# FYTalon/pienerf

Hardware: AMD Instinct MI355X
Metric: sim+render steps/s @800x800 chair (higher is better)
Workload: dtype f32 render / f64 sim

## Files before the change

### include/pienerf_hip.h

```cpp
#ifndef PIENERF_HIP_H
#define PIENERF_HIP_H
#include <stdint.h>
#ifdef __cplusplus
extern "C" {
#endif

#define PN_OK 0
#define PN_ERR_ARG 1
#define PN_ERR_HIP 2
#define PN_ERR_CAPACITY 3

const char* pn_version(void);

int pn_stream_create_cu_mask(uint32_t total_cu, uint32_t first_cu, uint32_t n_cu, int invert, void** stream_out);
int pn_stream_destroy(void* stream);
int pn_march_set_tail_rounds(int rounds);
int pn_march_set_skip_dda(int on);
int pn_device_cu_count(void);
const char* pn_last_error(void);


int pn_sph_from_ray(const float* rays_o, const float* rays_d, float radius, uint32_t N, float* coords, void* stream);
int pn_near_far_from_aabb(const float* rays_o, const float* rays_d, const float* aabb, uint32_t N, float min_near, float* nears, float* fars,
                          void* stream);
// ... 106 lines not shown
    float IP_dx;
    int cut;
    float cut_bounds[6];
    float bound;
    float min_near;
    float dt_gamma;
    uint32_t max_steps;
    float T_thresh;
    uint32_t cascade;
    uint32_t grid_size;
    float density_scale;
    float bg_color;
    int fp16;
    int reuse_tables;
    int ray_batch;
    int throughput;
    int throughput_trips;
    int ray_tile_w;
    int fused_from;
    int fused_whole;
    int fused_fold;
    int fused_grid;
    int fused_order;
} pn_render_opts;
int pn_frame_create(pn_frame** out, uint32_t max_rays, uint32_t max_vtx, uint32_t max_grid_cells);
void pn_frame_destroy(pn_frame* f);
int pn_render_deformed(pn_frame* f, const pn_net* net, const pn_render_opts* opts, const float* rays_o, const float* rays_d, uint32_t N,
                       const float* p_def, const float* p_ori, const float* F_IP, const float* dF_IP, int n_vtx, const uint8_t* bitfield,
                       float* image, float* depth, float* depth_0, float* weights_sum, int64_t* stats_host, void* stream);

int pn_render_deformed_async(pn_frame* f, const pn_net* net, const pn_render_opts* opts, const float* rays_o, const float* rays_d, uint32_t N,
                             const float* p_def, const float* p_ori, const float* F_IP, const float* dF_IP, int n_vtx, const uint8_t* bitfield,
                             float* image, float* depth, float* depth_0, float* weights_sum, int n_trips, void* stream);
int pn_render_status(pn_frame* f, int64_t* stats_host, int synchronize, void* stream);
int pn_frame_reset_unfinished(pn_frame* f, void* stream);

int pn_render_continue(pn_frame* f, const pn_net* net, const pn_render_opts* opts, const float* rays_o, const float* rays_d, uint32_t N,
                       const uint8_t* bitfield, float* image, float* depth, float* depth_0, float* weights_sum, int64_t* stats_host, int n_trips,
                       int is_static, void* stream);

int pn_render_static(pn_frame* f, const pn_net* net, const pn_render_opts* opts, const float* rays_o, const float* rays_d, uint32_t N,
                     const float* aabb_host, const uint8_t* bitfield, float* image, float* depth, float* depth_0, float* weights_sum,
                     int64_t* stats_host, int n_trips, void* stream);


typedef struct pn_copier pn_copier;
int pn_copier_create(pn_copier** out);
void pn_copier_destroy(pn_copier* c);
int pn_copier_submit(pn_copier* c, void* dst_host, const void* src_dev, uint64_t bytes, void* after_event, uint64_t* ticket);
int pn_copier_wait(pn_copier* c, uint64_t ticket);


int pn_mark_untrained_grid(const float* poses, uint32_t B, float fx, float fy, float cx, float cy, uint32_t cascade, uint32_t H, float bound,
                           float* density_grid, int* n_unseen, void* stream);
int pn_density_cells_full(uint32_t cascade, uint32_t H, float bound, const float* noise, float* xyzs, void* stream);
int pn_density_cells_partial(uint32_t cas, uint32_t H, float bound, uint32_t N, const int* rand_coords, const float* rand_pick, const float* noise,
                             const float* density_grid_cas, float* tmp_grid_cas, int* scratch, int* indices, float* xyzs, void* stream);
uint64_t pn_density_partial_scratch_ints(uint32_t H);
int pn_density_scatter(uint32_t n, const int* indices, const float* sigmas, float* tmp_grid_cas, void* stream);
int pn_density_grid_update(uint32_t n, float* density_grid, const float* tmp_grid, float decay, float density_thresh, uint8_t* bitfield,
                           double* partial, float* mean_thresh, void* stream);

int pn_frame_march_counters(pn_frame* f, int enable, uint64_t* counters_host, void* stream);
int pn_frame_fused_clocks(pn_frame* f, uint64_t* clocks_host, int* first_trip_out, int reset, void* stream);
int pn_fused_order_host(const float* rays_t, const float* fars, int n_rays, int* perm_out);
int pn_frame_trip_records(pn_frame* f, int* records_host, int* tail_counts_host, int max_trips, void* stream);
int pn_frame_trip_times(pn_frame* f, float* march_ms_host, float* network_ms_host, int max_trips, int* n_trips_out, void* stream);


int pn_sim_update_F(int n_IP, const int* topo, const double* dof, const double* Nx, const double* dNx, const double* ddNx, float* pos, float* F,
                    float* dF, void* stream);

int pn_sim_calc_elastic(int n_IP, const int* topo, const double* dNx, const double* dof, double* RF, double* VF, double* FF, int mcadams_sweeps,
                        void* stream);

int pn_sim_collect_rhs(int n_k, double dx, const int* csr_bg, const int* csr_cnt, const int* csr_buf, const double* mu, const double* lam,
                       const double* dNx, const double* RF, const double* VF, double* rhs, void* stream);

int pn_sim_matvec3(int n, const double* A, const double* X, double* Y, void* stream);

int pn_sim_stepforward(int n_k, int n_IP, int iters, double dt, double dx, const int* topo, const int* csr_bg, const int* csr_cnt,
                       const int* csr_buf, const double* mu, const double* lam, const double* dNx, const double* dNx_csr, const int* csr_pos,
                       const double* Ainv,
                       const double* Mmat, const double* dof_rest, const double* rhs_rest, const double* rhs_gravity, const double* dof_f,
                       double* dof, double* dof_vel, double* work, int prepared, int mcadams_sweeps, void* stream);
uint64_t pn_sim_work_doubles(int n_k, int n_IP);
int pn_sim_cells_chunk_ips(void);
// ... 248 lines not shown
```

### pienerf_amd/_lib.py

```python
import ctypes as C
import os

_HERE = os.path.dirname(os.path.abspath(__file__))
LIB_PATH = os.environ.get("PN_LIB_PATH") or os.path.join(_HERE, "lib", "libpienerf_hip.so")

P = C.c_void_p
u32, i32, f32, f64, u64 = C.c_uint32, C.c_int, C.c_float, C.c_double, C.c_uint64


class RenderOpts(C.Structure):
    _fields_ = [("max_iter_num", i32), ("hash_grid_size", f32), ("num_seek_IP", i32), ("IP_dx", f32), ("cut", i32), ("cut_bounds", f32 * 6),
                ("bound", f32), ("min_near", f32), ("dt_gamma", f32), ("max_steps", u32), ("T_thresh", f32), ("cascade", u32), ("grid_size", u32),
                ("density_scale", f32), ("bg_color", f32), ("fp16", i32), ("reuse_tables", i32), ("ray_batch", i32), ("throughput", i32), ("throughput_trips", i32), ("ray_tile_w", i32),
                ("fused_from", i32), ("fused_whole", i32), ("fused_fold", i32), ("fused_grid", i32), ("fused_order", i32)]


class ColliderStyle(C.Structure):
    _fields_ = [("rgb", (f32 * 3) * 8), ("checker", f32), ("checker_dim", f32), ("ambient", f32)]


class ShadowLight(C.Structure):
    _fields_ = [("c", f32 * 3), ("L", f32 * 3), ("U", f32 * 3), ("V", f32 * 3), ("half", f32), ("D", f32), ("S", i32), ("strength", f32), ("bias", f32),
                ("spheres", i32)]


class PointStyle(C.Structure):
    _fields_ = [("radius", i32), ("mode", i32), ("xray", i32), ("rgb", f32 * 3), ("ramp", (f32 * 3) * 3), ("lo", f32), ("hi", f32), ("alpha", f32),
                ("hidden_alpha", f32), ("bias", f32), ("marker_radius", f32), ("marker_thickness", f32)]


SIGNATURES = {
    "pn_version": (C.c_char_p, []),
    "pn_last_error": (C.c_char_p, []),
    "pn_stream_create_cu_mask": (i32, [u32, u32, u32, i32, C.POINTER(C.c_void_p)]),
    "pn_stream_destroy": (i32, [P]),
    "pn_device_cu_count": (i32, []),
    "pn_march_set_tail_rounds": (i32, [i32]),
# ... 43 lines not shown
    "pn_background_coords": (i32, [P, P, P, u32, P, i32, P]),
    "pn_nerf_color": (i32, [P, P, P, P, u32, P, P]),
    "pn_nerf_color_half": (i32, [P, P, P, P, u32, P, P]),
    "pn_render_hier": (i32, [P, P, P, u32, C.POINTER(f32), f32, i32, i32, f32, f32, P, P, P, P, i32, P]),
    "pn_hier_max_samples": (i32, []),
    "pn_frame_create": (i32, [C.POINTER(P), u32, u32, u32]),
    "pn_frame_destroy": (None, [P]),
    "pn_render_deformed": (i32, [P, P, C.POINTER(RenderOpts), P, P, u32, P, P, P, P, i32, P, P, P, P, P, P, P]),
    "pn_render_deformed_async": (i32, [P, P, C.POINTER(RenderOpts), P, P, u32, P, P, P, P, i32, P, P, P, P, P, i32, P]),
    "pn_render_status": (i32, [P, P, i32, P]),
    "pn_frame_reset_unfinished": (i32, [P, P]),
    "pn_render_continue": (i32, [P, P, C.POINTER(RenderOpts), P, P, u32, P, P, P, P, P, P, i32, i32, P]),
    "pn_render_static": (i32, [P, P, C.POINTER(RenderOpts), P, P, u32, P, P, P, P, P, P, P, i32, P]),
    "pn_mark_untrained_grid": (i32, [P, u32, f32, f32, f32, f32, u32, u32, f32, P, P, P]),
    "pn_density_cells_full": (i32, [u32, u32, f32, P, P, P]),
    "pn_density_cells_partial": (i32, [u32, u32, f32, u32, P, P, P, P, P, P, P, P, P]),
    "pn_density_partial_scratch_ints": (u64, [u32]),
    "pn_density_scatter": (i32, [u32, P, P, P, P]),
    "pn_density_grid_update": (i32, [u32, P, P, f32, f32, P, P, P, P]),
    "pn_frame_march_counters": (i32, [P, i32, P, P]),
    "pn_frame_trip_times": (i32, [P, P, P, i32, P, P]),
    "pn_frame_fused_clocks": (i32, [P, P, P, i32, P]),
    "pn_fused_order_host": (i32, [P, P, i32, P]),
    "pn_net_form": (i32, [P]),
    "pn_net_form_epoch": (i32, [P]),
    "pn_frame_trip_records": (i32, [P, P, P, i32, P]),
    "pn_sim_update_F": (i32, [i32, P, P, P, P, P, P, P, P, P]),
    "pn_sim_calc_elastic": (i32, [i32, P, P, P, P, P, P, i32, P]),
    "pn_sim_collect_rhs": (i32, [i32, f64, P, P, P, P, P, P, P, P, P, P]),
    "pn_sim_matvec3": (i32, [i32, P, P, P, P]),
    "pn_sim_stepforward": (i32, [i32, i32, i32, f64, f64, P, P, P, P, P, P, P, P, P, P, P, P, P, P, P, P, P, P, i32, i32, P]),
    "pn_sim_prepare": (i32, [i32, i32, P, P, P, P]),
    "pn_sim_cells_chunk_ips": (i32, []),
    "pn_sim_cells_work_doubles": (u64, [i32, i32]),
    "pn_sim_cells_prepare": (i32, [i32, i32, P, P]),
    "pn_sim_stepforward_cells": (i32, [i32, i32, i32, f64, f64, P, P, P, P, P, P, P, P, P, P, P, P, P, P, P, i32, P]),
    "pn_sim_bsr_matvec3": (i32, [i32, P, P, P, P, P, P]),
    "pn_sim_pcg_work_doubles": (u64, [i32]),
    "pn_sim_pcg_solve": (i32, [i32, P, P, P, P, P, P, P, f64, i32, P, P, P]),
    "pn_sim_stepforward_cells_pcg": (i32, [i32, i32, i32, f64, f64, P, P, P, P, P, P, P, P, P, P, P, P, f64, i32, P, P, P, P, P, P, P, P, P, i32, P]),
    "pn_sim_work_doubles": (u64, [i32, i32]),
    "pn_sim_coop_bytes": (u64, [i32, i32, i32]),
    "pn_sim_coop_prepare": (i32, [i32, i32, i32, P, P, P, C.POINTER(i32), P]),
    "pn_sim_coop_status": (i32, [P, C.POINTER(i32)]),
    "pn_sim_stepforward_coop": (i32, [i32, i32, i32, f64, f64, P, P, P, P, P, P, P, P, P, P, P, P, P, P, P, P, i32, C.POINTER(i32), P]),
    "pn_sim_update_force": (i32, [i32, i32, P, f64, P, P, P, P, P]),
# ... 98 lines not shown
```

### pienerf_amd/csrc/pn_render_ops.hip

```cpp
#include <float.h>

#include <vector>

#include "pn_render_records.h"
#include "pn_cell_hash.h"
#include "pn_side_tables.h"
#include "pn_march_kernels.h"
#include "pn_composite.h"
#include "pn_compact.h"
#include "pn_frame_kernels.h"

thread_local char pn_err_buf[512] = {0};

extern "C" int pn_device_cu_count(void) {
    int dev = 0, n = 0;
    if (hipGetDevice(&dev) != hipSuccess) return -1;
    if (hipDeviceGetAttribute(&n, hipDeviceAttributeMultiprocessorCount, dev) != hipSuccess) return -1;
    return n;
}

extern "C" int pn_stream_create_cu_mask(uint32_t total_cu, uint32_t first_cu, uint32_t n_cu, int invert, void** stream_out) {
    PN_REQUIRE(stream_out && total_cu > 0 && total_cu <= 1024 && n_cu > 0 && first_cu + n_cu <= total_cu);
    uint32_t mask[32];
    const uint32_t words = (total_cu + 31) / 32;
// ... 433 lines not shown
    pn_frame* f = c.f;
    const pn_net* net = c.net;
    const pn_render_opts* o = c.o;
    const bool whole = form == 1, fold = form == 2;
    int rc;
    if (fold) {
        if ((rc = time_mark(f, c.st, 0, 0, true))) return rc;
        enqueue_march(c, pl, 0, false);
        f->head_marched = 1;
        if ((rc = time_mark(f, c.st, 0, 1, true)) || (rc = time_mark(f, c.st, 0, 2, true))) return rc;
    }
    FusedArgs fa;
    memset(&fa, 0, sizeof(fa));
    fa.lv = (const PnFusedLevel*)(o->fp16 ? net->fused_levels : net->byte_levels); fa.emb = net->embeddings; fa.emb_h = (const uint32_t*)net->emb_half; fa.emb_bytes = net->n_entries * 4u;
    fa.wimg_g = (const uint4*)(o->fp16 ? net->whalf : (net->x_ok ? net->wx : net->wsplit)); fa.net_bound = net->bound; fa.net_inv2b = 1.0f / (2 * net->bound); fa.density_scale = o->density_scale;
    fa.x_scales = net->x_scales;
    fa.trips = f->trips + t; fa.N_rays = c.N; fa.max_steps = o->max_steps; fa.T_thresh = o->T_thresh;
    fa.alive = alive_list(f, t);
    fa.rays_t = f->rays_t; fa.weights_sum = c.weights_sum; fa.depth = c.depth_0; fa.image = f->acc_image;
    fa.xyzs = f->xyzs; fa.dirs = f->dirs; fa.deltas = f->deltas; fa.sigmas = f->sigmas; fa.rgbs = f->rgbs;
    fa.ctl = f->fused_ctl; fa.dev = f->dev; fa.tail_diag = f->tail_counts + t;
    fa.clocks = (f->march_counters_on & 4) ? f->fused_clocks : nullptr;
    fa.order = o->fused_order >= 0 ? 1 : 0;
    if (whole) {
        fa.active = f->active_seg; fa.active_counts = seg_counter(f, SEG_ACTIVE); fa.active_seg_cap = (int)f->seg_cap; fa.t_resume = f->t_resume;
        fa.blist = f->blist; fa.strag = f->strag; fa.blist_cap = f->blist_cap;
        fa.a_rounds = 24;
    }
    if (fold) {
        fa.list_seg = f->list_seg; fa.samp_counts = seg_counter(f, SEG_SAMP); fa.list_seg_cap = (int)f->seg_cap;
        fa.seg_tail = seg_counter(f, SEG_TAIL); fa.seg_back = seg_counter(f, SEG_BACK);
        fa.blist = f->blist; fa.strag = f->strag; fa.blist_cap = f->blist_cap;
    }
    if (finalize) {
        fa.finalize = 1; fa.bg = o->bg_color; fa.nears = f->nears; fa.fars_full = f->fars; fa.image_out = c.image; fa.depth_out = c.depth;
    }
    const int tb_idx = fold ? 1 : t;
    if ((rc = time_mark(f, c.st, tb_idx, 0, true))) return rc;
    if (whole) enqueue_skip(c, pl, make_march_io(c, pl, 0));
    const uint32_t blocks = o->fused_grid > 0 ? std::min((uint32_t)o->fused_grid, f->fused_blocks) : f->fused_blocks;
    rc = launch_trips_fused(o->num_seek_IP, o->max_iter_num > 1, o->fp16 ? 1 : (net->x_ok ? 2 : 0), form, blocks, c.st, c.mq, c.tb, fa);
    if (rc) return rc;
    if ((rc = time_mark(f, c.st, tb_idx, 1, true)) || (rc = time_mark(f, c.st, tb_idx, 2, true))) return rc;
    f->fused_first = tb_idx;
    f->fused_mode = form;
    return PN_OK;
// ... 161 lines not shown
            fprintf(stderr, "\n");
        }
#endif
        PN_HIP_CHECK(hipStreamSynchronize(st));
    }
    if ((enable & 1) && !(f->march_counters_on & 1)) PN_HIP_CHECK(hipMemsetAsync(f->march_counters, 0, 16 * sizeof(unsigned long long), st));
    f->march_counters_on = enable & 7;
    return PN_OK;
}

extern "C" int pn_frame_fused_clocks(pn_frame* f, uint64_t* clocks_host, int* first_trip_out, int reset, void* stream) {
    PN_REQUIRE(f);
    hipStream_t st = (hipStream_t)stream;
    if (clocks_host) {
        PN_HIP_CHECK(hipMemcpyAsync(clocks_host, f->fused_clocks, 16 * sizeof(unsigned long long), hipMemcpyDeviceToHost, st));
        PN_HIP_CHECK(hipStreamSynchronize(st));
        clocks_host[15] = f->fused_first >= 0 ? (uint64_t)f->fused_mode : 0u;
    }
    if (first_trip_out) *first_trip_out = f->fused_first;
    if (reset) PN_HIP_CHECK(hipMemsetAsync(f->fused_clocks, 0, 16 * sizeof(unsigned long long), st));
    return PN_OK;
}

extern "C" int pn_fused_order_host(const float* rays_t, const float* fars, int n_rays, int* perm_out) {
    PN_REQUIRE(n_rays >= 0 && (n_rays == 0 || (rays_t && fars && perm_out)));
    const int n_packets = (n_rays + PN_ORDER_PACKET - 1) / PN_ORDER_PACKET;
    const int n_ord = std::min(n_packets, PN_ORDER_CAP);
    std::vector<float> keys((size_t)n_ord, 0.0f);
    for (int k = 0; k < n_ord; k++)
        for (int s = 0; s < PN_ORDER_PACKET && k * PN_ORDER_PACKET + s < n_rays; s++)
            keys[k] = fmaxf(keys[k], pn_order_key(rays_t[k * PN_ORDER_PACKET + s], fars[k * PN_ORDER_PACKET + s]));
    for (int k = 0; k < n_ord; k++) perm_out[pn_order_rank(keys.data(), n_ord, k)] = k;
    for (int k = n_ord; k < n_packets; k++) perm_out[k] = k;
    return PN_OK;
}

extern "C" int pn_frame_trip_times(pn_frame* f, float* march_ms_host, float* network_ms_host, int max_trips, int* n_trips_out, void* stream) {
    PN_REQUIRE(f && march_ms_host && network_ms_host && n_trips_out && max_trips >= 0);
    PN_HIP_CHECK(hipStreamSynchronize((hipStream_t)stream));
    const int n = f->timed_trips < max_trips ? f->timed_trips : max_trips;
    if (f->stamped) {
        static unsigned long long host[PN_TIMED_TRIPS * 3];
        PN_HIP_CHECK(hipMemcpy(host, f->stamps, sizeof(unsigned long long) * (size_t)n * 3, hipMemcpyDeviceToHost));
        for (int t = 0; t < n; t++) {
            march_ms_host[t] = (float)((double)(host[t * 3 + 1] - host[t * 3]) * 1e-5);
            network_ms_host[t] = (float)((double)(host[t * 3 + 2] - host[t * 3 + 1]) * 1e-5);
// ... 40 lines not shown
```

### pienerf_amd/csrc/pn_trips_fused.h

```cpp
#pragma once
#define PN_TU_FP_CONTRACT_OFF 1
#include <cstddef>

#include "pn_net_tile.h"
#include "pn_fused_order.h"

#define PN_FUSED_MAX_TRIPS 128
#if PN_DBG_PHASES
#define PN_FUSED_PK , pk_dummy_
#else
#define PN_FUSED_PK
#endif
#ifndef PN_FUSED_WROUNDS
#define PN_FUSED_WROUNDS 1
#endif
#ifndef PN_FUSED_WAVES
#define PN_FUSED_WAVES 12
#endif
#ifndef PN_FUSED_LDS_OUT
#define PN_FUSED_LDS_OUT 1
#endif
#ifndef PN_FUSED_LDS_XYZ
#define PN_FUSED_LDS_XYZ 1
#endif
#define PN_FUSED_STAGE 512
#define PN_FUSED_CTL_HIST 0
#define PN_FUSED_CTL_DONE (PN_FUSED_CTL_HIST + 3 * PN_FUSED_MAX_TRIPS)
#define PN_FUSED_CTL_INTS (PN_FUSED_CTL_DONE + 32)
// ... 7 lines not shown
    float net_bound, net_inv2b, density_scale;
    const float* x_scales;
    PnTrip* trips;
    uint32_t N_rays, max_steps;
    float T_thresh;
    const int* alive;
    float *rays_t, *weights_sum, *depth, *image;
    float *xyzs, *dirs, *deltas, *sigmas, *rgbs;
    int* ctl;
    PnFrameDev* dev;
    int* tail_diag;
    unsigned long long* clocks;
    const int* active;
    const int* active_counts;
    int active_seg_cap;
    const float* t_resume;
    int* blist;
    int4* strag;
    uint32_t blist_cap;
    int a_rounds;
    int finalize; float bg; const float* nears; const float* fars_full; float* image_out; float* depth_out;
    const int* list_seg; const int* samp_counts; int list_seg_cap; const int* seg_tail; const int* seg_back;
    int order;
};

#ifndef PN_FUSED_FRESH_ARGS
#define PN_FUSED_FRESH_ARGS 1
#endif
__device__ __forceinline__ constexpr size_t pn_align_up(size_t v, size_t a) { return (v + a - 1) / a * a; }
template <typename T, int WHICH>
__device__ __forceinline__ const T& fused_karg_fresh(const T& by_value) {
#if PN_FUSED_FRESH_ARGS
    struct Layout { pnm::MarchParams a; pnm2::March2Tables tb; FusedArgs fa; };
    constexpr size_t off_tb = pn_align_up(sizeof(pnm::MarchParams), alignof(pnm2::March2Tables));
    constexpr size_t off_fa = pn_align_up(off_tb + sizeof(pnm2::March2Tables), alignof(FusedArgs));
    static_assert(off_tb == offsetof(Layout, tb) && off_fa == offsetof(Layout, fa), "kernarg placement of (MarchParams, March2Tables, FusedArgs)");
    constexpr size_t off = WHICH == 0 ? 0 : (WHICH == 1 ? off_tb : off_fa);
    uint32_t z;
    asm volatile("s_mov_b32 %0, 0" : "=s"(z));
    const char __attribute__((address_space(4)))* kp = (const char __attribute__((address_space(4)))*)__builtin_amdgcn_kernarg_segment_ptr();
    return *reinterpret_cast<const T*>((const char*)kp + off + z);
#else
    return by_value;
#endif
}
__device__ __forceinline__ const FusedArgs& fused_args_fresh(const FusedArgs& by_value) { return fused_karg_fresh<FusedArgs, 2>(by_value); }
// ... 66 lines not shown
#define PN_FUSED_ACHUNK 64
#endif

template <int K, bool MULTI, int NF, int MODE>
__global__ void __launch_bounds__(PN_FUSED_WAVES * 64, (PN_FUSED_WAVES + 3) / 4) k_trips_fused(pnm::MarchParams a, pnm2::March2Tables tb, FusedArgs fa) {
    extern __shared__ __attribute__((aligned(16))) uint4 fused_lds[];
    constexpr bool HALF = NF == 1, XF = NF == 2;
    constexpr int IMG16 = (HALF ? PN_NET_HALF_BYTES : (XF ? PN_NET_X_BYTES : PN_NET_SPLIT_BYTES)) / 16;
    constexpr int MAXT = PN_FUSED_MAX_TRIPS;
    constexpr int AC = PN_FUSED_ACHUNK;
    static_assert(AC == 64 || AC == 32, "rays per first-trip chunk");
    constexpr bool WHOLE = MODE == 1;
    constexpr bool FOLD = MODE == 2;
    constexpr bool QUEUED = MODE != 0;
    uint4* wimg = fused_lds;
    float4* stage_all = reinterpret_cast<float4*>(fused_lds + IMG16 + 32);
    int* hist = reinterpret_cast<int*>(stage_all + PN_FUSED_WAVES * PN_FUSED_STAGE);
    constexpr bool LXYZ = PN_FUSED_LDS_XYZ != 0 && PN_FUSED_LDS_OUT != 0 && NF != 0;
    float* xyz_all = reinterpret_cast<float*>(hist + 3 * MAXT);
    __shared__ int s_last, s_cursor;
    __shared__ int s_bres, s_bready, s_bhead, s_sres, s_sready, s_shead, s_pending, s_a1done;
    __shared__ int s_pend[PN_FUSED_MAXCHUNKS];
    __shared__ int s_pref[PN_SEGS + 1];
    __shared__ unsigned short s_perm[PN_ORDER_CAP];

#if PN_DBG_PHASES
    pnm3::PhaseClock pk_dummy_;
#endif
    const PnTrip* tr = fa.trips;
    const int lane = threadIdx.x & 63, wv = threadIdx.x >> 6;
    if (PN_FUSED_FRESH_ARGS && blockIdx.x == 0 && threadIdx.x == 0) {
        const FusedArgs& fk = fused_args_fresh(fa);
        const pnm::MarchParams& ak = fused_karg_fresh<pnm::MarchParams, 0>(a);
        const pnm2::March2Tables& tk = fused_karg_fresh<pnm2::March2Tables, 1>(tb);
        if (fk.trips != fa.trips || fk.rays_t != fa.rays_t || fk.N_rays != fa.N_rays || fk.image_out != fa.image_out || fk.seg_back != fa.seg_back || ak.rays_o != a.rays_o ||
            ak.grid != a.grid || ak.hgs != a.hgs || tk.nb != tb.nb || tk.rec != tb.rec) atomicOr(&fa.dev->err, 32);
    }
    const float x_scale = XF ? fa.x_scales[0] : 1.0f, x_rscale = XF ? fa.x_scales[1] : 1.0f;
    int A = 0, sb0 = 0, n_active = 0;
    if (QUEUED) {
        if (threadIdx.x < 64) {
            const int cnt = seg_count(WHOLE ? fa.active_counts : fa.samp_counts, lane);
            int inc = cnt;
#pragma unroll
            for (int o = 1; o < 64; o <<= 1) {
                const int u = __shfl_up(inc, o);
                if (lane >= o) inc += u;
            }
            s_pref[lane + 1] = inc;
            if (lane == 0) s_pref[0] = 0;
        }
        __syncthreads();
        n_active = s_pref[PN_SEGS];
        const long long chunks = ((long long)n_active + AC - 1) / AC;
        const bool ok = tr->n_alive == (int)fa.N_rays && tr->n_step == 1 && tr->step_base == 0 && (long long)n_active * 8 <= (long long)fa.N_rays &&
                        (chunks + (long long)gridDim.x) * AC <= (long long)fa.blist_cap &&
                        (WHOLE ? (chunks + (long long)gridDim.x - 1) / (long long)gridDim.x <= PN_FUSED_MAXCHUNKS : true);
        if (!ok) return;
        sb0 = 1;
    } else {
        A = tr->n_alive; sb0 = tr->step_base;
        if (!(A > 0 && tr->n_step == 8 && tr->dense != 0)) return;
    }

    for (int i = threadIdx.x; i < IMG16; i += PN_FUSED_WAVES * 64) wimg[i] = fa.wimg_g[i];
    if (threadIdx.x < 16 * sizeof(PnFusedLevel) / 16) wimg[IMG16 + threadIdx.x] = reinterpret_cast<const uint4*>(fa.lv)[threadIdx.x];
    for (int i = threadIdx.x; i < 3 * MAXT; i += PN_FUSED_WAVES * 64) hist[i] = 0;
    if (threadIdx.x == 0) { s_cursor = 0; s_bres = s_bready = s_bhead = s_sres = s_sready = s_shead = s_a1done = 0; }
    if (QUEUED) {
        const int n_items0 = WHOLE ? (n_active + AC - 1) / AC : (n_active + 31) / 32;
        const int mine0 = (int)blockIdx.x < n_items0 ? (n_items0 - (int)blockIdx.x + (int)gridDim.x - 1) / (int)gridDim.x : 0;
        if (threadIdx.x == 0) s_pending = mine0;
        if (WHOLE)
            for (int i = threadIdx.x; i < PN_FUSED_MAXCHUNKS; i += PN_FUSED_WAVES * 64) s_pend[i] = 64;
    }
    __syncthreads();

    const int sub = lane & 7, gbase = lane & ~7, grp = lane >> 3;
    const uint32_t wave_g = blockIdx.x * PN_FUSED_WAVES + wv;
    const uint32_t slotw = (FOLD ? fa.N_rays : 0u) + wave_g * 64u, slot0 = slotw + (uint32_t)grp * 8u;
    float4* stage = stage_all + wv * PN_FUSED_STAGE;
    const uint4* __restrict__ wl = wimg + lane;
    const int half = lane >> 5, s32 = lane & 31;
    const PnFusedLevel* lds_lv = reinterpret_cast<const PnFusedLevel*>(wimg + IMG16) + 8 * half;
    __amdgpu_buffer_rsrc_t emb_rsrc = __builtin_amdgcn_make_buffer_rsrc(const_cast<uint32_t*>(fa.emb_h), 0, (int)fa.emb_bytes, 0x00020000);
    float* const X = LXYZ ? xyz_all + wv * 192 + grp * 24 : fa.xyzs + (size_t)slot0 * 3;
    float* const Dd = LXYZ ? nullptr : fa.dirs + (size_t)slot0 * 3;
    float* const dl = fa.deltas + (size_t)slot0 * 2;

    const bool clk = fa.clocks != nullptr;
    unsigned long long c_acc[10] = {0, 0, 0, 0, 0, 0, 0, 0, 0, 0}, c_t = 0, rounds = 0;
    auto tick = [&](int k) __attribute__((always_inline)) {
        if (clk) {
            asm volatile("s_waitcnt vmcnt(0) lgkmcnt(0)" ::: "memory");
            const unsigned long long n = __builtin_readcyclecounter();
            c_acc[k] += n - c_t;
            c_t = n;
        }
    };
    unsigned long long rt0 = 0;
    if (clk) { c_t = __builtin_readcyclecounter(); rt0 = __builtin_amdgcn_s_memrealtime(); }

    float r_ox = 0.f, r_oy = 0.f, r_oz = 0.f, r_dx = 1.f, r_dy = 1.f, r_dz = 1.f, r_rdx = 1.f, r_rdy = 1.f, r_rdz = 1.f, r_far = 0.f, r_t = 0.f;
    auto network_tile = [&](uint32_t slot, float4* lds_out = nullptr, const float* lds_xyz = nullptr, int dir_lane = 0) __attribute__((always_inline)) {
        pnm3::Float3 p, d;
        if (LXYZ && lds_xyz) {
            p = *reinterpret_cast<const pnm3::Float3*>(lds_xyz);
            d.x = __shfl(r_dx, dir_lane); d.y = __shfl(r_dy, dir_lane); d.z = __shfl(r_dz, dir_lane);
        } else {
            p = *reinterpret_cast<const pnm3::Float3*>(fa.xyzs + (size_t)slot * 3);
            d = *reinterpret_cast<const pnm3::Float3*>(fa.dirs + (size_t)slot * 3);
        }
        float sigma_logit, e[3];
        if (HALF) {
            float g2[8];
            tile_sigma_net_h<4>(fa.lv, wimg, emb_rsrc, wl, half, fa.net_bound, p.x, p.y, p.z, g2);
            sigma_logit = g2[0];
            __builtin_amdgcn_sched_barrier(0);
            tile_color_net_h(wl, wimg, half, g2, d.x, d.y, d.z, e);
        } else if (XF) {
            const f32x16 h2 = tile_sigma_net_x<PN_BF_LU>(reinterpret_cast<const PnByteLevel*>(lds_lv), fa.emb, wl, half, fa.net_bound, fa.net_inv2b, p.x, p.y, p.z, x_scale);
            sigma_logit = h2[0] * x_rscale;
            __builtin_amdgcn_sched_barrier(0);
            tile_color_net_x(wl, wimg, half, h2, d.x, d.y, d.z, e);
        } else {
            const f32x16 h2 = tile_sigma_net<PN_BF_LU>(reinterpret_cast<const PnByteLevel*>(lds_lv), fa.emb, wl, half, fa.net_bound, fa.net_inv2b, p.x, p.y, p.z);
            sigma_logit = h2[0];
            __builtin_amdgcn_sched_barrier(0);
            tile_color_net(wl, wimg, half, h2, d.x, d.y, d.z, e);
        }
        if (half == 0) {
            const float sg_ = tile_sigma_out(fa.density_scale, sigma_logit);
            const float c0_ = HALF ? tile_rgb_out_h(e[0]) : tile_rgb_out(e[0]), c1_ = HALF ? tile_rgb_out_h(e[1]) : tile_rgb_out(e[1]),
                        c2_ = HALF ? tile_rgb_out_h(e[2]) : tile_rgb_out(e[2]);
            if (lds_out) {
                *lds_out = make_float4(sg_, c0_, c1_, c2_);
            } else {
                fa.sigmas[slot] = sg_;
                fa.rgbs[(size_t)slot * 3] = c0_; fa.rgbs[(size_t)slot * 3 + 1] = c1_; fa.rgbs[(size_t)slot * 3 + 2] = c2_;
            }
        }
    };
    auto network64 = [&](unsigned long long rm, bool own = true, uint32_t lane_slot = 0u) __attribute__((always_inline)) {
#pragma unroll 1
        for (int tile = 0; tile < 2; tile++) {
            if (!((rm >> (32 * tile)) & 0xFFFFFFFFull)) continue;
            network_tile(own ? slotw + 32u * (uint32_t)tile + (uint32_t)s32 : lane_slot, (PN_FUSED_LDS_OUT && own) ? stage + 32 * tile + s32 : nullptr,
                         (LXYZ && own) ? xyz_all + wv * 192 + (32 * tile + s32) * 3 : nullptr, (4 * tile + (s32 >> 3)) * 8);
        }
    };
    auto wave_sync_mem = [&]() __attribute__((always_inline)) {
        __builtin_amdgcn_fence(__ATOMIC_RELEASE, "workgroup");
        asm volatile("s_waitcnt vmcnt(0)" ::: "memory");
        __builtin_amdgcn_fence(__ATOMIC_ACQUIRE, "workgroup");
    };

    int share = 0;
    const int* my_list = nullptr;
    int my_chunks = 0;
    int *a_index = nullptr, *blist = nullptr;
    int4* strag = nullptr;
    uint32_t a_base = 0;
    bool go_on = true;
    auto lds_ld = [](int* p_) __attribute__((always_inline)) { return __hip_atomic_load(p_, __ATOMIC_RELAXED, __HIP_MEMORY_SCOPE_WORKGROUP); };
    auto lds_st = [](int* p_, int v) __attribute__((always_inline)) { __hip_atomic_store(p_, v, __ATOMIC_RELAXED, __HIP_MEMORY_SCOPE_WORKGROUP); };
    auto q_claim = [&](int* head, int* ready, int want, int& take) __attribute__((always_inline)) {
        int base = 0;
        take = 0;
        for (;;) {
            const int h = lds_ld(head), r = lds_ld(ready);
            const int t_ = min(want, r - h);
            if (t_ <= 0) break;
            if (atomicCAS(head, h, h + t_) == h) { base = h; take = t_; break; }
        }
        return base;
    };
    auto q_publish = [&](int* ready, int base, int n) __attribute__((always_inline)) {
        while (lds_ld(ready) != base) __builtin_amdgcn_s_sleep(1);
        lds_st(ready, base + n);
    };
    auto chunk_finish = [&](int ci) __attribute__((always_inline)) {
#pragma unroll 1
        for (int tile = 0; tile < AC / 32; tile++) {
            const int pos = ci * AC + tile * 32 + s32;
            const uint32_t slot = a_base + (uint32_t)pos;
            const bool has = fa.deltas[(size_t)slot * 2] != 0.0f;
            const unsigned long long em = __ballot(has && half == 0);
            if (!em) continue;
            if (lane == 0) {
                atomicAdd(&hist[MAXT], (int)__popcll(em));
                if (a.stats) atomicAdd(a.stats + 3, (unsigned long long)__popcll(em));
            }
            network_tile(slot);
            wave_sync_mem();
            tick(7);
            bool on = false;
            int idx = -1;
            if (has && half == 0) {
                idx = a_index[pos];
                on = composite_one(idx, slot, 1u, fa.T_thresh, fa.rays_t, fa.sigmas, fa.rgbs, fa.deltas, fa.weights_sum, fa.depth, fa.image) && go_on;
                if (!on && fa.finalize) finalize_ray(fa, idx);
            }
            const unsigned long long om = __ballot(on);
            wave_sync_mem();
            if (om) {
                int base = 0;
                if (lane == 0) base = atomicAdd(&s_bres, (int)__popcll(om));
                base = __builtin_amdgcn_readfirstlane(base);
                if (on) blist[base + (int)__popcll(om & ((1ull << lane) - 1ull))] = idx;
                wave_sync_mem();
                if (lane == 0) q_publish(&s_bready, base, (int)__popcll(om));
            }
            tick(8);
        }
        if (lane == 0) atomicSub(&s_pending, 1);
// ... 174 lines not shown
                    f_has = e < n_active;
                    if (f_has) {
                        int lo = 0, hi = PN_SEGS;
                        while (hi - lo > 1) {
                            const int mid = (lo + hi) >> 1;
                            if (s_pref[mid] <= e) lo = mid; else hi = mid;
                        }
                        f_slot = (uint32_t)fa.list_seg[(size_t)lo * fa.list_seg_cap + (e - s_pref[lo])];
                    }
                    f_slot = f_has ? f_slot : (uint32_t)__builtin_amdgcn_readlane((int)f_slot, (int)__builtin_ctzll(__ballot(f_has)));
                }
            }
            if (!fold_round) {
                int fin = 0;
                if (lane == 0) fin = (lds_ld(&s_pending) == 0 && lds_ld(&s_bhead) >= lds_ld(&s_bready)) ? 1 : 0;
                if (__builtin_amdgcn_readfirstlane(fin)) break;
                __builtin_amdgcn_s_sleep(32);
                tick(9);
                continue;
            }
        }
        unsigned long long net_mask = 0ull;
        bool have_ray = false;
        if (fold_round) {
            net_mask = __ballot(f_has && half == 0);
            if (lane == 0) atomicAdd(&hist[MAXT], (int)__popcll(net_mask));
            tick(0);
        } else {
        rounds++;
        tick(0);
        have_ray = index >= 0;
        if (have_ray && sub == 0) atomicAdd(&hist[j], 1);
        const pnm::MarchParams& am = fused_karg_fresh<pnm::MarchParams, 0>(a);
        const pnm2::March2Tables& tbm = fused_karg_fresh<pnm2::March2Tables, 1>(tb);
        pnm3::RayConsts c;
        pnm3::frame_consts(am, c);
        c.ox = r_ox; c.oy = r_oy; c.oz = r_oz; c.dx = r_dx; c.dy = r_dy; c.dz = r_dz; c.rdx = r_rdx; c.rdy = r_rdy; c.rdz = r_rdz; c.far = r_far;
        pnm3::RayState st{0.f, 0.f, 0u};
        bool have = false;
        if (have_ray) {
            float t = r_t;
            t += pnm::clampf(t * am.dt_gamma, c.dt_min, c.dt_max) * 0.0f;
            st.last_t = t;
            st.t = t;
            have = t < c.far;
        }
        const bool done = pnm3::march_window<K, MULTI, 8, PN_FUSED_STAGE, 1>(am, tbm, c, 8u, sub, gbase, lane, stage, X, Dd, dl, st, PN_FUSED_WROUNDS, have PN_FUSED_PK);
        const bool deferred = have && !done;
// ... 7 lines not shown
            pnm3::frame_consts(am, c2);
            c2.ox = readlane_f(c.ox, L); c2.oy = readlane_f(c.oy, L); c2.oz = readlane_f(c.oz, L);
            c2.dx = readlane_f(c.dx, L); c2.dy = readlane_f(c.dy, L); c2.dz = readlane_f(c.dz, L);
            c2.rdx = readlane_f(c.rdx, L); c2.rdy = readlane_f(c.rdy, L); c2.rdz = readlane_f(c.rdz, L);
            c2.far = readlane_f(c.far, L);
            pnm3::RayState s2{readlane_f(st.t, L), readlane_f(st.last_t, L), (uint32_t)__builtin_amdgcn_readlane((int)st.step, L)};
            const size_t sl = (size_t)slotw + (size_t)(L >> 3) * 8;
            pnm3::march_window<K, MULTI, 64, PN_FUSED_STAGE, 1>(am, tbm, c2, 8u, lane, 0, lane, stage, LXYZ ? xyz_all + wv * 192 + (L >> 3) * 24 : fa.xyzs + sl * 3,
                                                                LXYZ ? nullptr : fa.dirs + sl * 3, fa.deltas + sl * 2, s2, 0x7fffffff, true PN_FUSED_PK);
            if (gbase == L) st.step = s2.step;
        }
        const uint32_t emitted = have_ray ? st.step : 0u;
        if (have_ray && sub == 0 && emitted) {
            atomicAdd(&hist[MAXT + j], (int)emitted);
            if (a.stats) atomicAdd(a.stats + 3, (unsigned long long)emitted);
        }
        if (have_ray && (uint32_t)sub >= emitted) {
            dl[2 * sub] = 0.0f; dl[2 * sub + 1] = 0.0f;
            X[3 * sub] = X[3 * sub + 1] = X[3 * sub + 2] = 0.0f;
            if (!LXYZ) Dd[3 * sub] = Dd[3 * sub + 1] = Dd[3 * sub + 2] = 0.0f;
        }
        wave_sync_mem();
        tick(2);
        net_mask = __ballot(have_ray);
        }
        network64(net_mask, !fold_round, f_slot);
        wave_sync_mem();
        tick(fold_round ? 7 : 3);
        if (fold_round) {
            bool on = false;
            int idx = -1;
            if (f_has && half == 0) {
                idx = fa.alive[f_slot];
                on = composite_one(idx, f_slot, 1u, fa.T_thresh, fa.rays_t, fa.sigmas, fa.rgbs, fa.deltas, fa.weights_sum, fa.depth, fa.image) && go_on;
                if (!on && fa.finalize) finalize_ray(fa, idx);
            }
            const unsigned long long om = __ballot(on);
            wave_sync_mem();
            if (om) {
                int base = 0;
                if (lane == 0) base = atomicAdd(&s_bres, (int)__popcll(om));
                base = __builtin_amdgcn_readfirstlane(base);
                if (on) blist[base + (int)__popcll(om & ((1ull << lane) - 1ull))] = idx;
                wave_sync_mem();
                if (lane == 0) q_publish(&s_bready, base, (int)__popcll(om));
            }
            if (lane == 0) atomicSub(&s_pending, 1);
            tick(8);
            continue;
// ... 6 lines not shown
        alive = __shfl(alive, gbase);
        r_t = __shfl(r_t, gbase);
        if (have_ray) {
            if (alive && (uint32_t)(sb0 + 8 * (j + (QUEUED ? 0 : 1))) < fa.max_steps && j + 1 < MAXT) j++;
            else {
                if (QUEUED && fc.finalize && sub == 0) finalize_ray(fc, index);
                index = -1;
            }
        }
        tick(4);
    }
    if (clk && lane == 0) {
        for (int k = 0; k < 5; k++) atomicAdd(fa.clocks + k, c_acc[k]);
        atomicAdd(fa.clocks + 5, rounds);
        atomicAdd(fa.clocks + 6, 1ull);
        atomicAdd(fa.clocks + 7, __builtin_amdgcn_s_memrealtime() - rt0);
        atomicMax(fa.clocks + 8, rounds);
        atomicMax(fa.clocks + 9, __builtin_amdgcn_s_memrealtime() - rt0);
        if (QUEUED)
            for (int k = 5; k < 10; k++) atomicAdd(fa.clocks + 5 + k, c_acc[k]);
    }

    __syncthreads();
    for (int i = threadIdx.x; i < 3 * MAXT; i += PN_FUSED_WAVES * 64) {
        const int v = hist[i];
        if (v) atomicAdd(fa.ctl + PN_FUSED_CTL_HIST + i, v);
    }
    asm volatile("s_waitcnt vmcnt(0)" ::: "memory");
    __syncthreads();
    if (threadIdx.x == 0) {
        const int old = atomicAdd(fa.ctl + PN_FUSED_CTL_DONE, 1);
        s_last = (old == (int)gridDim.x - 1) ? 1 : 0;
    }
    __syncthreads();
    if (!s_last || threadIdx.x >= 64) return;
    int m = 0;
    long long n_samples_total = 0;
    for (int j0 = 0; j0 < MAXT; j0 += 64) {
        const int jj = j0 + lane;
        int* hp = fa.ctl + PN_FUSED_CTL_HIST + jj;
        int al = __hip_atomic_load(hp, __ATOMIC_RELAXED, __HIP_MEMORY_SCOPE_AGENT);
        const int em = __hip_atomic_load(hp + MAXT, __ATOMIC_RELAXED, __HIP_MEMORY_SCOPE_AGENT);
        const int tl = __hip_atomic_load(hp + 2 * MAXT, __ATOMIC_RELAXED, __HIP_MEMORY_SCOPE_AGENT);
        if (QUEUED && jj == 0) al = (int)fa.N_rays;
        m += (int)__popcll(__ballot(al > 0));
        {
// ... 79 lines not shown
```

### pienerf_amd/nerf/frame_hooks.py

```python
import ctypes as C

from .._lib import check, lib, stream_ptr


class FrameHooksMixin:
    def march_counters(self, enable, read=False, slot=0):
        out = (C.c_uint64 * 4)() if read else None
        check(lib().pn_frame_march_counters(self._frames[slot][0], int(enable), out, stream_ptr()), "march_counters")
        return None if out is None else dict(iterations=int(out[0]), candidates=int(out[1]), warps=int(out[2]), samples=int(out[3]))

    def fused_clocks(self, slot=0, reset=False):
        out, first = (C.c_uint64 * 16)(), C.c_int(-1)
        check(lib().pn_frame_fused_clocks(self._frames[slot][0], out, C.byref(first), int(bool(reset)), stream_ptr()), "fused_clocks")
        return dict(refill=int(out[0]), march=int(out[1]), windows=int(out[2]), network=int(out[3]), composite=int(out[4]), wave_rounds=int(out[5]),
                    waves=int(out[6]), lifetime_ticks=int(out[7]), max_rounds=int(out[8]), max_lifetime_ticks=int(out[9]), first_trip=int(first.value),
                    a_march=int(out[10]), a_windows=int(out[11]), a_network=int(out[12]), a_composite=int(out[13]), a_barrier=int(out[14]),
                    mode=int(out[15]))

    def trip_records(self, slot=0, max_trips=16):
        rec, tail = (C.c_int * (5 * max_trips))(), (C.c_int * max_trips)()
        check(lib().pn_frame_trip_records(self._frames[slot][0], rec, tail, max_trips, stream_ptr()), "trip_records")
        return [tuple(rec[5 * i:5 * i + 5]) + (tail[i],) for i in range(max_trips) if rec[5 * i] > 0]

    def trip_times(self, slot=0):
        a, b, n = (C.c_float * 64)(), (C.c_float * 64)(), C.c_int(0)
        check(lib().pn_frame_trip_times(self._frames[slot][0], a, b, 64, C.byref(n), stream_ptr()), "trip_times")
        return [float(a[i]) for i in range(n.value)], [float(b[i]) for i in range(n.value)]
```

### pienerf_amd/nerf/renderer.py

```python
import ctypes as C
import math

import torch
import torch.nn as nn

from .._lib import RenderOpts, check, lib, ptr, require_gpu, stream_ptr
from ._outputs import flat_rays, frame_outputs
from .frame_hooks import FrameHooksMixin
from .overlay_colliders import ColliderOverlayMixin
from .overlay_points import PointOverlayMixin
from .render_deformed_ops import DeformedOpsMixin
from .render_hier import HierRenderMixin, sample_pdf
from .render_static import StaticRenderMixin


def frame_background(bg_color, bg_radius, overlay):
    if bg_radius > 0:
        return 0.0, 0.0, None
    if bg_color is None:
        bg_color = 1
    if torch.is_tensor(bg_color):
        return 0.0, 0.0, bg_color
    return (0.0 if overlay else bg_color), bg_color, None

# ... 91 lines not shown
        o.max_iter_num = int(kwargs.get("max_iter_num"))
        o.hash_grid_size = float(kwargs.get("hash_grid_size"))
        o.num_seek_IP = int(kwargs.get("num_seek_IP"))
        o.IP_dx = float(self.IP_dx)
        o.cut = int(bool(kwargs.get("cut")))
        cb = kwargs.get("cut_bounds") or [0.0] * 6
        for i in range(6):
            o.cut_bounds[i] = float(cb[i])
        o.bound = float(kwargs.get("bound", self.bound))
        o.reuse_tables = int(bool(kwargs.get("reuse_tables")))
        o.ray_batch = int(kwargs.get("ray_batch") or 0)
        o.throughput = int(kwargs.get("march_throughput") or 0)
        o.throughput_trips = int(kwargs.get("march_throughput_trips") or 0)
        tw = kwargs.get("ray_tile_w")
        if tw is None and n_rays and kwargs.get("W") and kwargs.get("H") and int(kwargs["W"]) * int(kwargs["H"]) == n_rays:
            tw = kwargs["W"]
        o.ray_tile_w = int(tw or 0)
        o.fused_from = int(kwargs.get("fused_from") or 0)
        o.fused_grid = int(kwargs.get("fused_grid") or 0)
        o.fused_fold = int(bool(kwargs.get("fused_fold")))
        o.fused_whole = int(bool(kwargs.get("fused_whole")))
        fo = kwargs.get("fused_order")
        o.fused_order = 0 if (fo is None or fo) else -1
        return o

    def rund_cuda(self, rays_o, rays_d, dt_gamma=0, bg_color=None, perturb=False, max_steps=1024, T_thresh=1e-2, _shadow_pass=False, **kwargs):
        if perturb:
            self._refuse_overlays("the op-by-op loop (perturb=True)")
            return self.rund_cuda_ops(rays_o, rays_d, dt_gamma, bg_color, perturb, max_steps, T_thresh, **kwargs)
        prefix = rays_o.shape[:-1]
        rays_o, rays_d = flat_rays(rays_o, rays_d)
        require_gpu(rays_o, rays_d)
        N, device = rays_o.shape[0], rays_o.device
        overlay = self._overlay is not None and not _shadow_pass
        bg_driver, bg_colliders, bg_tensor = frame_background(bg_color, self.bg_radius, overlay)
        if bg_tensor is not None:
            bg_tensor = bg_tensor.to(device=device, dtype=torch.float32)
        p_def, p_ori, F_IP, dF_IP = self._ip_state(device)
        assert p_def.shape == p_ori.shape and p_ori.shape[0] > 0
        n_vtx = p_ori.shape[0]
        if overlay and self._shadows is not None:
            self._render_shadow_map(dt_gamma, max_steps, T_thresh, kwargs)
        o = self._deformed_opts(dt_gamma, bg_driver, max_steps, T_thresh, kwargs, n_rays=N)
        ob = kwargs.get("out_buffers")
        image, depth, depth_0, weights_sum = frame_outputs(N, device, ob)
        async_trips, slot = int(kwargs.get("async_trips") or 0), int(kwargs.get("frame_slot") or 0)
# ... 81 lines not shown
```

Before: 1511.

## Compact sparse fused network tiles into one tile via lane-group select

In the fused march/network kernel, waves whose active rays span both 32-lane halves but occupy at most four 8-lane groups are remapped so a single network tile covers them, and rays that emitted no samples are dropped from the network mask. This aims to cut redundant MLP tile evaluations when few samples are live. The change adds select-mask arithmetic, LDS indirection for slot lookup, and optional tile counters behind the clocks flag. It is on by default through the new fused_thin option.

Result: no change. 1504 (-0.5%).

```diff
diff --git a/include/pienerf_hip.h b/include/pienerf_hip.h
--- a/include/pienerf_hip.h
+++ b/include/pienerf_hip.h
@@ -152,6 +152,7 @@
     int fused_fold;
     int fused_grid;
     int fused_order;
+    int fused_thin;
 } pn_render_opts;
 int pn_frame_create(pn_frame** out, uint32_t max_rays, uint32_t max_vtx, uint32_t max_grid_cells);
 void pn_frame_destroy(pn_frame* f);
@@ -193,6 +194,8 @@
 
 int pn_frame_march_counters(pn_frame* f, int enable, uint64_t* counters_host, void* stream);
 int pn_frame_fused_clocks(pn_frame* f, uint64_t* clocks_host, int* first_trip_out, int reset, void* stream);
+int pn_frame_fused_tiles(pn_frame* f, uint64_t* tiles_host, void* stream);
+int pn_fused_thin_host(int mask8, int* out4);
 int pn_fused_order_host(const float* rays_t, const float* fars, int n_rays, int* perm_out);
 int pn_frame_trip_records(pn_frame* f, int* records_host, int* tail_counts_host, int max_trips, void* stream);
 int pn_frame_trip_times(pn_frame* f, float* march_ms_host, float* network_ms_host, int max_trips, int* n_trips_out, void* stream);
diff --git a/pienerf_amd/_lib.py b/pienerf_amd/_lib.py
--- a/pienerf_amd/_lib.py
+++ b/pienerf_amd/_lib.py
@@ -12,7 +12,7 @@
     _fields_ = [("max_iter_num", i32), ("hash_grid_size", f32), ("num_seek_IP", i32), ("IP_dx", f32), ("cut", i32), ("cut_bounds", f32 * 6),
                 ("bound", f32), ("min_near", f32), ("dt_gamma", f32), ("max_steps", u32), ("T_thresh", f32), ("cascade", u32), ("grid_size", u32),
                 ("density_scale", f32), ("bg_color", f32), ("fp16", i32), ("reuse_tables", i32), ("ray_batch", i32), ("throughput", i32), ("throughput_trips", i32), ("ray_tile_w", i32),
-                ("fused_from", i32), ("fused_whole", i32), ("fused_fold", i32), ("fused_grid", i32), ("fused_order", i32)]
+                ("fused_from", i32), ("fused_whole", i32), ("fused_fold", i32), ("fused_grid", i32), ("fused_order", i32), ("fused_thin", i32)]
 
 
 class ColliderStyle(C.Structure):
@@ -102,6 +102,8 @@
     "pn_frame_trip_times": (i32, [P, P, P, i32, P, P]),
     "pn_frame_fused_clocks": (i32, [P, P, P, i32, P]),
     "pn_fused_order_host": (i32, [P, P, i32, P]),
+    "pn_frame_fused_tiles": (i32, [P, P, P]),
+    "pn_fused_thin_host": (i32, [i32, P]),
     "pn_net_form": (i32, [P]),
     "pn_net_form_epoch": (i32, [P]),
     "pn_frame_trip_records": (i32, [P, P, P, i32, P]),
diff --git a/pienerf_amd/csrc/pn_fused_thin.h b/pienerf_amd/csrc/pn_fused_thin.h
--- /dev/null
+++ b/pienerf_amd/csrc/pn_fused_thin.h
@@ -0,0 +1,32 @@
+#pragma once
+#include <cstdint>
+
+#if defined(__HIPCC__) || defined(__CUDACC__)
+#define PN_THIN_HD __host__ __device__ __forceinline__
+#else
+#define PN_THIN_HD inline
+#endif
+
+#define PN_THIN_SEL_LO 0x03020100u
+#define PN_THIN_SEL_HI 0x07060504u
+
+PN_THIN_HD int pn_thin_ctz8(uint32_t m) { return __builtin_ctz(m); }
+
+PN_THIN_HD int pn_thin_select(uint32_t mask8, uint32_t* sel) {
+    uint32_t m = mask8 & 0xFFu;
+    if (!m) return 0;
+    const uint32_t p0 = (uint32_t)pn_thin_ctz8(m);
+    uint32_t s = p0 * 0x01010101u;
+    int n = 1;
+    m &= m - 1u;
+    for (int v = 1; v < 4 && m; v++) {
+        s = (s & ~(0xFFu << (8 * v))) | ((uint32_t)pn_thin_ctz8(m) << (8 * v));
+        m &= m - 1u;
+        n++;
+    }
+    if (m) return 0;
+    *sel = s;
+    return n;
+}
+
+PN_THIN_HD bool pn_thin_needed(uint32_t mask8) { return (mask8 & 0x0Fu) != 0u && (mask8 & 0xF0u) != 0u; }
diff --git a/pienerf_amd/csrc/pn_render_ops.hip b/pienerf_amd/csrc/pn_render_ops.hip
--- a/pienerf_amd/csrc/pn_render_ops.hip
+++ b/pienerf_amd/csrc/pn_render_ops.hip
@@ -479,6 +479,7 @@
     fa.ctl = f->fused_ctl; fa.dev = f->dev; fa.tail_diag = f->tail_counts + t;
     fa.clocks = (f->march_counters_on & 4) ? f->fused_clocks : nullptr;
     fa.order = o->fused_order >= 0 ? 1 : 0;
+    fa.thin = o->fused_thin >= 0 ? 1 : 0;
     if (whole) {
         fa.active = f->active_seg; fa.active_counts = seg_counter(f, SEG_ACTIVE); fa.active_seg_cap = (int)f->seg_cap; fa.t_resume = f->t_resume;
         fa.blist = f->blist; fa.strag = f->strag; fa.blist_cap = f->blist_cap;
@@ -686,6 +687,25 @@
     return PN_OK;
 }
 
+extern "C" int pn_frame_fused_tiles(pn_frame* f, uint64_t* tiles_host, void* stream) {
+    PN_REQUIRE(f && tiles_host);
+    hipStream_t st = (hipStream_t)stream;
+    unsigned long long w = 0;
+    PN_HIP_CHECK(hipMemcpyAsync(&w, f->fused_clocks + 15, sizeof(w), hipMemcpyDeviceToHost, st));
+    PN_HIP_CHECK(hipStreamSynchronize(st));
+    tiles_host[0] = w & 0xFFFFFFFFull;
+    tiles_host[1] = w >> 32;
+    return PN_OK;
+}
+
+extern "C" int pn_fused_thin_host(int mask8, int* out4) {
+    uint32_t sel = 0;
+    const int n = pn_thin_select((uint32_t)mask8, &sel);
+    if (n == 0 || !out4) return 0;
+    for (int v = 0; v < 4; v++) out4[v] = (int)((sel >> (8 * v)) & 0xFFu);
+    return pn_thin_needed((uint32_t)mask8) ? n : -n;
+}
+
 extern "C" int pn_fused_order_host(const float* rays_t, const float* fars, int n_rays, int* perm_out) {
     PN_REQUIRE(n_rays >= 0 && (n_rays == 0 || (rays_t && fars && perm_out)));
     const int n_packets = (n_rays + PN_ORDER_PACKET - 1) / PN_ORDER_PACKET;
diff --git a/pienerf_amd/csrc/pn_trips_fused.h b/pienerf_amd/csrc/pn_trips_fused.h
--- a/pienerf_amd/csrc/pn_trips_fused.h
+++ b/pienerf_amd/csrc/pn_trips_fused.h
@@ -4,6 +4,7 @@
 
 #include "pn_net_tile.h"
 #include "pn_fused_order.h"
+#include "pn_fused_thin.h"
 
 #define PN_FUSED_MAX_TRIPS 128
 #if PN_DBG_PHASES
@@ -57,6 +58,7 @@
     int finalize; float bg; const float* nears; const float* fars_full; float* image_out; float* depth_out;
     const int* list_seg; const int* samp_counts; int list_seg_cap; const int* seg_tail; const int* seg_back;
     int order;
+    int thin;
 };
 
 #ifndef PN_FUSED_FRESH_ARGS
@@ -169,6 +171,7 @@
     __shared__ int s_bres, s_bready, s_bhead, s_sres, s_sready, s_shead, s_pending, s_a1done;
     __shared__ int s_pend[PN_FUSED_MAXCHUNKS];
     __shared__ int s_pref[PN_SEGS + 1];
+    __shared__ unsigned s_tiles[2];
     __shared__ unsigned short s_perm[PN_ORDER_CAP];
 
 #if PN_DBG_PHASES
@@ -213,7 +216,7 @@
     for (int i = threadIdx.x; i < IMG16; i += PN_FUSED_WAVES * 64) wimg[i] = fa.wimg_g[i];
     if (threadIdx.x < 16 * sizeof(PnFusedLevel) / 16) wimg[IMG16 + threadIdx.x] = reinterpret_cast<const uint4*>(fa.lv)[threadIdx.x];
     for (int i = threadIdx.x; i < 3 * MAXT; i += PN_FUSED_WAVES * 64) hist[i] = 0;
-    if (threadIdx.x == 0) { s_cursor = 0; s_bres = s_bready = s_bhead = s_sres = s_sready = s_shead = s_a1done = 0; }
+    if (threadIdx.x == 0) { s_tiles[0] = s_tiles[1] = 0u; s_cursor = 0; s_bres = s_bready = s_bhead = s_sres = s_sready = s_shead = s_a1done = 0; }
     if (QUEUED) {
         const int n_items0 = WHOLE ? (n_active + AC - 1) / AC : (n_active + 31) / 32;
         const int mine0 = (int)blockIdx.x < n_items0 ? (n_items0 - (int)blockIdx.x + (int)gridDim.x - 1) / (int)gridDim.x : 0;
@@ -249,12 +252,20 @@
     if (clk) { c_t = __builtin_readcyclecounter(); rt0 = __builtin_amdgcn_s_memrealtime(); }
 
     float r_ox = 0.f, r_oy = 0.f, r_oz = 0.f, r_dx = 1.f, r_dy = 1.f, r_dz = 1.f, r_rdx = 1.f, r_rdy = 1.f, r_rdz = 1.f, r_far = 0.f, r_t = 0.f;
-    auto network_tile = [&](uint32_t slot, float4* lds_out = nullptr, const float* lds_xyz = nullptr, int dir_lane = 0) __attribute__((always_inline)) {
+    auto sel_slot = [&](uint32_t sel) __attribute__((always_inline)) {
+        int gb = gbase;
+        asm volatile("" : "+v"(gb));
+        return ((sel >> (gb & 24)) & 0xFFu) * 8u + (uint32_t)sub;
+    };
+    auto network_tile = [&](uint32_t slot, bool own = false, uint32_t sel = 0u) __attribute__((always_inline)) {
         pnm3::Float3 p, d;
-        if (LXYZ && lds_xyz) {
-            p = *reinterpret_cast<const pnm3::Float3*>(lds_xyz);
+        if (LXYZ && own) {
+            const uint32_t ls = sel_slot(sel);
+            const int dir_lane = (int)(ls & ~7u);
+            p = *reinterpret_cast<const pnm3::Float3*>(xyz_all + wv * 192 + ls * 3);
             d.x = __shfl(r_dx, dir_lane); d.y = __shfl(r_dy, dir_lane); d.z = __shfl(r_dz, dir_lane);
         } else {
+            if (own) slot = slotw + sel_slot(sel);
             p = *reinterpret_cast<const pnm3::Float3*>(fa.xyzs + (size_t)slot * 3);
             d = *reinterpret_cast<const pnm3::Float3*>(fa.dirs + (size_t)slot * 3);
         }
@@ -280,20 +291,29 @@
             const float sg_ = tile_sigma_out(fa.density_scale, sigma_logit);
             const float c0_ = HALF ? tile_rgb_out_h(e[0]) : tile_rgb_out(e[0]), c1_ = HALF ? tile_rgb_out_h(e[1]) : tile_rgb_out(e[1]),
                         c2_ = HALF ? tile_rgb_out_h(e[2]) : tile_rgb_out(e[2]);
-            if (lds_out) {
-                *lds_out = make_float4(sg_, c0_, c1_, c2_);
+            if (PN_FUSED_LDS_OUT && own) {
+                asm volatile("" : "+s"(sel));
+                stage[sel_slot(sel)] = make_float4(sg_, c0_, c1_, c2_);
             } else {
+                if (own) { asm volatile("" : "+s"(sel)); slot = slotw + sel_slot(sel); }
                 fa.sigmas[slot] = sg_;
                 fa.rgbs[(size_t)slot * 3] = c0_; fa.rgbs[(size_t)slot * 3 + 1] = c1_; fa.rgbs[(size_t)slot * 3 + 2] = c2_;
             }
         }
     };
-    auto network64 = [&](unsigned long long rm, bool own = true, uint32_t lane_slot = 0u) __attribute__((always_inline)) {
+    auto network64 = [&](unsigned long long rm, bool own = true, uint32_t lane_slot = 0u, bool thin_on = false) __attribute__((always_inline)) {
+        uint32_t sel0 = PN_THIN_SEL_LO;
+        uint32_t run = ((uint32_t)rm != 0u ? 1u : 0u) | ((uint32_t)(rm >> 32) != 0u ? 2u : 0u);
+        if (own && thin_on) {
+            const uint32_t gm = (uint32_t)(((rm & 0x0101010101010101ull) * 0x0102040810204080ull) >> 56);
+            uint32_t s_ = PN_THIN_SEL_LO;
+            if (pn_thin_needed(gm) && pn_thin_select(gm, &s_) != 0) { sel0 = s_; run = 1u; }
+        }
 #pragma unroll 1
         for (int tile = 0; tile < 2; tile++) {
-            if (!((rm >> (32 * tile)) & 0xFFFFFFFFull)) continue;
-            network_tile(own ? slotw + 32u * (uint32_t)tile + (uint32_t)s32 : lane_slot, (PN_FUSED_LDS_OUT && own) ? stage + 32 * tile + s32 : nullptr,
-                         (LXYZ && own) ? xyz_all + wv * 192 + (32 * tile + s32) * 3 : nullptr, (4 * tile + (s32 >> 3)) * 8);
+            if (!((run >> tile) & 1u)) continue;
+            if (clk && lane == 0) atomicAdd(&s_tiles[0], 1u);
+            network_tile(lane_slot, own, tile ? PN_THIN_SEL_HI : sel0);
         }
     };
     auto wave_sync_mem = [&]() __attribute__((always_inline)) {
@@ -338,6 +358,7 @@
                 atomicAdd(&hist[MAXT], (int)__popcll(em));
                 if (a.stats) atomicAdd(a.stats + 3, (unsigned long long)__popcll(em));
             }
+            if (clk && lane == 0) { atomicAdd(&s_tiles[0], 1u); atomicAdd(&s_tiles[1], 1u); }
             network_tile(slot);
             wave_sync_mem();
             tick(7);
@@ -558,8 +579,10 @@
         }
         unsigned long long net_mask = 0ull;
         bool have_ray = false;
+        const bool thin_on = fused_args_fresh(fa).thin != 0;
         if (fold_round) {
             net_mask = __ballot(f_has && half == 0);
+            if (clk && lane == 0) atomicAdd(&s_tiles[1], 1u);
             if (lane == 0) atomicAdd(&hist[MAXT], (int)__popcll(net_mask));
             tick(0);
         } else {
@@ -613,9 +636,13 @@
         }
         wave_sync_mem();
         tick(2);
-        net_mask = __ballot(have_ray);
-        }
-        network64(net_mask, !fold_round, f_slot);
+        net_mask = __ballot(have_ray && (emitted != 0u || !thin_on));
+        if (clk) {
+            const unsigned long long pm = __ballot(have_ray);
+            if (lane == 0) atomicAdd(&s_tiles[1], ((uint32_t)pm != 0u ? 1u : 0u) + ((uint32_t)(pm >> 32) != 0u ? 1u : 0u));
+        }
+        }
+        network64(net_mask, !fold_round, f_slot, thin_on);
         wave_sync_mem();
         tick(fold_round ? 7 : 3);
         if (fold_round) {
@@ -668,6 +695,7 @@
     }
 
     __syncthreads();
+    if (clk && threadIdx.x == 0) atomicAdd(fa.clocks + 15, ((unsigned long long)s_tiles[1] << 32) | (unsigned long long)s_tiles[0]);
     for (int i = threadIdx.x; i < 3 * MAXT; i += PN_FUSED_WAVES * 64) {
         const int v = hist[i];
         if (v) atomicAdd(fa.ctl + PN_FUSED_CTL_HIST + i, v);
diff --git a/pienerf_amd/nerf/frame_hooks.py b/pienerf_amd/nerf/frame_hooks.py
--- a/pienerf_amd/nerf/frame_hooks.py
+++ b/pienerf_amd/nerf/frame_hooks.py
@@ -10,12 +10,14 @@
         return None if out is None else dict(iterations=int(out[0]), candidates=int(out[1]), warps=int(out[2]), samples=int(out[3]))
 
     def fused_clocks(self, slot=0, reset=False):
-        out, first = (C.c_uint64 * 16)(), C.c_int(-1)
+        out, first, tiles = (C.c_uint64 * 16)(), C.c_int(-1), (C.c_uint64 * 2)()
+        check(lib().pn_frame_fused_tiles(self._frames[slot][0], tiles, stream_ptr()), "fused_tiles")
         check(lib().pn_frame_fused_clocks(self._frames[slot][0], out, C.byref(first), int(bool(reset)), stream_ptr()), "fused_clocks")
         return dict(refill=int(out[0]), march=int(out[1]), windows=int(out[2]), network=int(out[3]), composite=int(out[4]), wave_rounds=int(out[5]),
                     waves=int(out[6]), lifetime_ticks=int(out[7]), max_rounds=int(out[8]), max_lifetime_ticks=int(out[9]), first_trip=int(first.value),
                     a_march=int(out[10]), a_windows=int(out[11]), a_network=int(out[12]), a_composite=int(out[13]), a_barrier=int(out[14]),
-                    mode=int(out[15]))
+                    mode=int(out[15]),
+                    tiles=int(tiles[0]), tiles_plain=int(tiles[1]))
 
     def trip_records(self, slot=0, max_trips=16):
         rec, tail = (C.c_int * (5 * max_trips))(), (C.c_int * max_trips)()
diff --git a/pienerf_amd/nerf/renderer.py b/pienerf_amd/nerf/renderer.py
--- a/pienerf_amd/nerf/renderer.py
+++ b/pienerf_amd/nerf/renderer.py
@@ -137,6 +137,8 @@
         o.fused_whole = int(bool(kwargs.get("fused_whole")))
         fo = kwargs.get("fused_order")
         o.fused_order = 0 if (fo is None or fo) else -1
+        ft = kwargs.get("fused_thin")
+        o.fused_thin = 0 if (ft is None or ft) else -1
         return o
 
     def rund_cuda(self, rays_o, rays_d, dt_gamma=0, bg_color=None, perturb=False, max_steps=1024, T_thresh=1e-2, _shadow_pass=False, **kwargs):
```
